# CrispyChillies/Image-Retrieval---Thesis-2026

Measured on AMD Instinct MI355X. Metric: queries/sec (embed+top-10) over 1M x 1024 gallery, higher is better.
Workload: dtype f32 embed (two fp16 MFMA terms); bf16 MFMA candidates + f64 re-rank

## Files before the change

image-retrieval---thesis-2026_amd/_lib.py:

```python
import ctypes
import os

_HERE = os.path.dirname(os.path.abspath(__file__))
LIB_PATH = os.environ.get("MIRX_LIB_PATH", os.path.join(_HERE, "libmirx.so"))

METRIC_IP = 0
ESTATE = -4
METRIC_NEG_L2 = 1
TIER_AUTO = 0
TIER_EXACT_ONLY = 3
OPT_TIERS = 1
OPT_SAMPLE_RANK = 2
OPT_FORCE_TAU = 3
OPT_PROFILE = 4
OPT_RANK_SORT = 5
OPT_COMPACT_CHUNK_ROWS = 6
OPT_MASK_GATHER_BYTES = 7
OPT_RANGE_MAX_HITS = 8
RANK_SORT_AUTO = 0
RANK_SORT_BITONIC = 1
RANK_SORT_RADIX = 2
MAX_SEARCH_K = 1024
GROUP_MAX_LIMIT, GROUP_MAX_SIZE, GROUP_MAX_HITS, GROUP_FILL_MAX = 1024, 64, 16384, 4096
FUSE_MAX_REQUESTS, FUSE_MAX_ENTRIES, FUSE_MAX_LIMIT = 8, 4096, 1024
FUSE_RRF, FUSE_WEIGHTED = 0, 1
FUSE_NORMS = {"RAW": 0, "COSINE": 1, "IP": 2, "L2": 3}
TUNE_CONV1X1_SMALL_MAX_WG = 1
TUNE_CONV3X3_SMALL_MAX_WG = 2
TUNE_CONV1X1_RING = 3
SIMCAM_MAPS_BOTH = 0
SIMCAM_MAPS_RETRIEVED = 1
SIMATT_GROUP = 0
SIMATT_PAIRS = 1
ANOMALY_BAD_SCORE = 1
ANOMALY_BAD_NORM = 2
ANOMALY_BAD_ONE_CLASS = 4
ANOMALY_BAD_EMPTY_CLASS = 8
RESAMPLE_MAX_SIDE = 8192
RESAMPLE_MAX_TAPS = 65
RESAMPLE_MAX_OUT = 1024
RESAMPLE_MAX_BATCH = 65536
RESAMPLE_MAX_LDS = 65536
RESAMPLE_TILE_W, RESAMPLE_TILE_H = 32, 16
RESAMPLE_DESC_WORDS = 8
RESAMPLE_OUT_U8, RESAMPLE_OUT_F32 = 0, 1
RESAMPLE_BILINEAR, RESAMPLE_BICUBIC = 0, 1
IVF_MAX_NLIST, IVF_MAX_DIM = 65536, 2048
IVF_FLAT, IVF_SQ8 = 0, 1
IVF_PQ = 2
PQ_MAX_M = 64
IVF_OPT_SCORE_BYTES = 1
ROLLOUT_FUSE = {"mean": 0, "max": 1, "min": 2}
STAGES = ("prep", "sample", "gemm", "finalize", "exact")
FORCE_TAU_OFF = 0x7FC00000


class MirxError(RuntimeError):
    """A libmirx call failed (message from mirx_last_error())."""


class SearchStats(ctypes.Structure):
    _fields_ = [(n, ctypes.c_int64) for n in
                ("nq", "tier1_answered", "exact_answered", "candidates", "reranked",
                 "overflowed", "incomplete", "left_out")]

    def as_dict(self):
        return {n: int(getattr(self, n)) for n, _ in self._fields_}


class RangeStats(ctypes.Structure):
    _fields_ = [(n, ctypes.c_int64) for n in ("nq", "filter_answered", "exact_answered", "candidates", "hits")]

    def as_dict(self):
        return {n: int(getattr(self, n)) for n, _ in self._fields_}


class IvfStats(ctypes.Structure):
    _fields_ = [(n, ctypes.c_int64) for n in ("nq", "rows_scored", "pairs", "work_items", "batches")]

    def as_dict(self):
        return {n: int(getattr(self, n)) for n, _ in self._fields_}


_vp, _i64, _int = ctypes.c_void_p, ctypes.c_int64, ctypes.c_int
SYMBOLS = {
    "mirx_last_error": (ctypes.c_char_p, []),
    "mirx_version": (_int, []),
    "mirx_set_tuning": (_int, [_int, _i64]),
    "mirx_index_create": (_int, [_int, _int, _int, ctypes.POINTER(_vp)]),
    "mirx_index_destroy": (None, [_vp]),
    "mirx_index_add": (_int, [_vp, _vp, _i64, _vp]),
    "mirx_index_reserve": (_int, [_vp, _i64]),
    "mirx_index_size": (_i64, [_vp]),
    "mirx_index_dim": (_int, [_vp]),
    "mirx_index_set_option": (_int, [_vp, _int, _i64]),
    "mirx_index_get_rows": (_int, [_vp, _i64, _i64, _vp, _vp]),
    "mirx_index_remove_ids": (_int, [_vp, _vp, _i64, ctypes.POINTER(_i64), _vp]),
    "mirx_compact_tile": (_int, []),
    "mirx_index_search": (_int, [_vp, _vp, _i64, _int, _vp, _vp, _vp, _vp]),
    "mirx_index_search_f64": (_int, [_vp, _vp, _i64, _int, _vp, _vp, _vp, _vp]),
    "mirx_index_search_begin": (_int, [_vp, _vp, _i64, _int, _vp, _vp, _vp, _vp, _vp]),
    "mirx_index_search_end": (_int, [_vp]),
    "mirx_index_search_masked": (_int, [_vp, _vp, _i64, _int, _vp, _vp, _i64, _vp, _vp, _vp, _vp]),
    "mirx_index_search_deep": (_int, [_vp, _vp, _i64, _int, _vp, _vp, _vp, _vp, _vp, _vp]),
    "mirx_index_search_leave_out": (_int, [_vp, _vp, _i64, _int, _vp, _vp, _vp, _vp, _i64, _vp, _vp, _vp, _vp]),
    "mirx_tier1_max_k": (_int, []),
    "mirx_deep_min_rows": (_i64, [_int, _i64]),
    "mirx_index_rank_top_masked": (_int, [_vp, _vp, _i64, _i64, _vp, _vp, _i64, _vp, _vp, _vp, _vp]),
    "mirx_index_range_search": (_int, [_vp, _vp, _i64, ctypes.c_double, ctypes.c_double, _vp, _vp, _i64, _vp,
                                       ctypes.POINTER(_i64), _vp]),
    "mirx_index_range_fetch": (_int, [_vp, _vp, _vp, _vp, _vp]),
    "mirx_index_range_last_stats": (_int, [_vp, ctypes.POINTER(RangeStats)]),
# ... 201 lines not shown
```

image-retrieval---thesis-2026_amd/csrc/k_stem_h2.hip:

```cpp
#include "mirx_device.h"
#include "mirx_kernels.h"

namespace mirx {

namespace {

constexpr int PTH = 8, PTW = 7;
constexpr int CTH = 2 * PTH + 1;
constexpr int CTW = 2 * PTW + 1;
constexpr int NPX = CTH * CTW;
constexpr int ITH = 2 * (CTH - 1) + 7;
constexpr int ITW = 2 * (CTW - 1) + 7;
constexpr int PH = 24;
constexpr int PLANE = 3 * ITH * PH;
constexpr int OCB = 32;
constexpr int NOB = 2;
constexpr int NSTEP = 11;
constexpr int CONV_PITCH = 260;
constexpr int S_IN = 2 * PLANE;
constexpr int S_CONV = OCB * CONV_PITCH;
constexpr int W_BYTES = NOB * NSTEP * 2 * OCB * 16 * 2;
constexpr int STEP_BYTES = NOB * 2 * 1024;
constexpr int RING_OFF = S_IN * 4;
#if defined(MIRX_STEM_NCH) && !defined(MIRX_DIAG)
#error "MIRX_STEM_NCH without -DMIRX_DIAG: the shipped library carries one ring depth"
#endif
#ifndef MIRX_STEM_NCH
#define MIRX_STEM_NCH 2
#endif
constexpr int par_off(int nch) { return RING_OFF + 2 * nch * STEP_BYTES; }
constexpr int lds_bytes(int nch) { return par_off(nch) + 4 * NOB * OCB * 4; }
constexpr int wg_per_cu(int nch) { return 160 * 1024 / lds_bytes(nch) > 4 ? 4 : 160 * 1024 / lds_bytes(nch); }
static_assert(lds_bytes(2) <= 40960, "NCH = 2: four workgroups per CU");

__device__ inline void split2h_pair_cvt(float a, float b, unsigned &h, unsigned &l) {
    const f32x2 v = {a, b};
    const f16x2 vh = __builtin_convertvector(v, f16x2);
    const f32x2 r1 = v - __builtin_convertvector(vh, f32x2);
    const f16x2 vl = __builtin_convertvector(r1, f16x2);
    h = __builtin_bit_cast(unsigned, vh);
    l = __builtin_bit_cast(unsigned, vl);
}

template <typename TIN, int NCH>
__global__ __launch_bounds__(256, wg_per_cu(NCH)) void k_stem_h2(const TIN *__restrict__ x, const uint16_t *__restrict__ w3,
                                                                 const float *__restrict__ oscale, const float *__restrict__ scale,
                                                                 const float *__restrict__ shift, int h, int wd,
                                                                 float *__restrict__ y, int64_t y_bs,
                                                                 const float *__restrict__ in_range, unsigned *__restrict__ out_range,
                                                                 const float *__restrict__ mean, const float *__restrict__ stdv) {
    extern __shared__ __attribute__((aligned(16))) float sm[];
    constexpr bool U8 = sizeof(TIN) == 1;
    constexpr int NCHUNK = (NSTEP + NCH - 1) / NCH;
    constexpr int RING_BUF = NCH * STEP_BYTES;
    constexpr int PAR_OFF = par_off(NCH);
    static_assert(S_CONV * 4 <= PAR_OFF, "the conv tile of a channel block lies over the patch and the ring");
    static_assert(!U8 || 768 * 4 <= RING_BUF, "the 8-bit table lies in ring buffer 1");
    char *s_ring = reinterpret_cast<char *>(sm) + RING_OFF;
    float *s_lut = reinterpret_cast<float *>(s_ring + RING_BUF);
    if (U8) {
        for (int i = threadIdx.x; i < 768; i += 256) s_lut[i] = ((float)(i & 255) / 255.0f - mean[i >> 8]) / stdv[i >> 8];
        __syncthreads();
    }
    float *s_in = sm;
    float *s_conv = sm;
    const int ph = h / 4, pw = wd / 4, ch = h / 2, cw = wd / 2;
    const int tiles_x = (pw + PTW - 1) / PTW;
    int tile = blockIdx.x;
    int64_t img = blockIdx.y;
#ifndef MIRX_STEM_PLAIN_ORDER
    {
        const unsigned ntile = gridDim.x, lin = blockIdx.x + ntile * blockIdx.y, full = gridDim.y & ~7u;
        if (lin < ntile * full) {
            const unsigned j = lin >> 3;
            tile = (int)(j % ntile);
            img = (int64_t)(j / ntile) * 8 + (lin & 7);
        }
    }
#endif
    const int tile_y = tile / tiles_x, tile_x = tile % tiles_x;
    const int oc0 = 0;
    const int py0 = tile_y * PTH, px0 = tile_x * PTW;
    const int cy0 = 2 * py0 - 1, cx0 = 2 * px0 - 1;
    const int iy0 = 2 * cy0 - 3, ix0 = 2 * cx0 - 3;
    const TIN *xi = x + img * 3 * (int64_t)h * wd;
    float x_scale, x_inv;
    range_scales(in_range[img], x_scale, x_inv);
    float *s_par = sm + PAR_OFF / 4;
    if (threadIdx.x < NOB * OCB) {
        s_par[4 * threadIdx.x] = oscale[threadIdx.x] * x_inv;
        s_par[4 * threadIdx.x + 1] = scale[threadIdx.x];
        s_par[4 * threadIdx.x + 2] = shift[threadIdx.x];
    }

#ifndef MIRX_STEM_EXP
#define MIRX_STEM_EXP 0
#endif
    const int dwv = __builtin_amdgcn_readfirstlane(threadIdx.x >> 6);
    const __amdgpu_buffer_rsrc_t wrsrc = __builtin_amdgcn_make_buffer_rsrc((void *)w3, 0, W_BYTES, 0x00020000);
    const int dvoff = ((threadIdx.x & 63) >> 1) * 32 + (((threadIdx.x & 1) ^ ((threadIdx.x >> 4) & 1)) << 4);
    auto issue_chunk = [&](int c) {
        if (MIRX_STEM_EXP & 8) return;
#pragma unroll
        for (int j = 0; j < NCH; ++j) {
            const int s = c * NCH + j;
            if (s < NSTEP)
                __builtin_amdgcn_raw_ptr_buffer_load_lds(wrsrc, LDS_PTR(s_ring + (c & 1) * RING_BUF + j * STEP_BYTES + dwv * 1024), 16,
                                                         dvoff, ((dwv >> 1) * NSTEP * 2 + s * 2 + (dwv & 1)) * 1024, 0, 0);
        }
    };
    issue_chunk(0);
    if (!U8 && NCHUNK > 1) issue_chunk(1);

    constexpr int ROWW = 36, RPP = 7;
    constexpr int N_IN = (3 * ITH + RPP - 1) / RPP;
    const int s_row = threadIdx.x / ROWW, s_q = threadIdx.x % ROWW;
    const int xx = ix0 + s_q;
    const bool col_ok = s_row < RPP && s_q < ITW && xx >= 0 && xx < wd;
    const bool lane_live = s_row < RPP;
    float vin[N_IN];
#pragma unroll
    for (int t = 0; t < N_IN; ++t) {
        const int row = RPP * t + s_row;
        const int c = (row >= ITH) + (row >= 2 * ITH), r = row - c * ITH;
        const int yy = iy0 + r;
        vin[t] = 0.0f;
        if (col_ok && row < 3 * ITH && yy >= 0 && yy < h) {
            if constexpr (U8) vin[t] = s_lut[c * 256 + xi[((int64_t)c * h + yy) * wd + xx]];
            else vin[t] = xi[((int64_t)c * h + yy) * wd + xx];
        }
    }
    unsigned *s_w = reinterpret_cast<unsigned *>(s_in);
    const int s_dst = (s_q & 1) * PLANE + s_row * PH + (s_q >> 1);
#pragma unroll
    for (int t = 0; t < N_IN; ++t) {
        const float v = vin[t] * x_scale;
        const _Float16 vh = (_Float16)v;
        const _Float16 vl = (_Float16)(v - (float)vh);
        const unsigned word = (unsigned)__builtin_bit_cast(unsigned short, vh) | ((unsigned)__builtin_bit_cast(unsigned short, vl) << 16);
        if (lane_live && RPP * t + s_row < 3 * ITH) s_w[s_dst + RPP * t * PH] = word;
    }
    asm volatile("s_waitcnt vmcnt(0)" ::: "memory");
    __syncthreads();
    if (U8 && NCHUNK > 1) issue_chunk(1);

    const int wave = threadIdx.x >> 6, lane = threadIdx.x & 63;
    const int half = lane >> 5, n = lane & 31;
    int xbase[2];
#pragma unroll
    for (int t = 0; t < 2; ++t) {
        int p = (2 * wave + t) * 32 + n;
        if (p >= NPX) p = NPX - 1;
        const int r = p / CTW, q = p % CTW;
        xbase[t] = 2 * r * PH + q;
    }
    const char *wp = s_ring + n * 32 + ((half ^ ((n >> 3) & 1)) << 4);
    f32x16 acc[2][NOB];
#pragma unroll
    for (int t = 0; t < 2; ++t)
#pragma unroll
        for (int b = 0; b < NOB; ++b)
#pragma unroll
            for (int r = 0; r < 16; ++r) acc[t][b][r] = 0.0f;
#pragma unroll
    for (int c = 0; c < ((MIRX_STEM_EXP & 1) ? 0 : NCHUNK); ++c) {
        if (c > 0 && c + 1 < NCHUNK) issue_chunk(c + 1);
        __builtin_amdgcn_sched_barrier(0);
        const char *wc = wp + (c & 1) * RING_BUF;
#pragma unroll
        for (int j = 0; j < NCH; ++j) {
            const int s = c * NCH + j;
            if (s >= NSTEP) break;
            f16x8 ah[NOB], al[NOB];
#pragma unroll
            for (int b = 0; b < NOB; ++b) {
                ah[b] = *reinterpret_cast<const f16x8 *>(wc + j * STEP_BYTES + (b * 2 + 0) * 1024);
                al[b] = *reinterpret_cast<const f16x8 *>(wc + j * STEP_BYTES + (b * 2 + 1) * 1024);
            }
            const int rho0 = 2 * s, rho1 = 2 * s + 1 < 21 ? 2 * s + 1 : 20;
            const int ro0 = ((rho0 / 7) * ITH + rho0 % 7) * PH, ro1 = ((rho1 / 7) * ITH + rho1 % 7) * PH;
            const int ro = half ? ro1 : ro0;
#pragma unroll
            for (int t = 0; t < 2; ++t) {
                const unsigned *pe = s_w + xbase[t] + ro;
                const unsigned *po = pe + PLANE;
                u32x4 bh, bl;
                bh[0] = __builtin_amdgcn_perm(pe[1], pe[0], 0x05040100u); bl[0] = __builtin_amdgcn_perm(pe[1], pe[0], 0x07060302u);
                bh[1] = __builtin_amdgcn_perm(pe[3], pe[2], 0x05040100u); bl[1] = __builtin_amdgcn_perm(pe[3], pe[2], 0x07060302u);
                bh[2] = __builtin_amdgcn_perm(po[1], po[0], 0x05040100u); bl[2] = __builtin_amdgcn_perm(po[1], po[0], 0x07060302u);
                bh[3] = __builtin_amdgcn_perm(po[3], po[2], 0x05040100u); bl[3] = __builtin_amdgcn_perm(po[3], po[2], 0x07060302u);
                const f16x8 xh = __builtin_bit_cast(f16x8, bh), xl = __builtin_bit_cast(f16x8, bl);
#pragma unroll
                for (int b = 0; b < NOB; ++b) {
                    f32x16 a3 = acc[t][b];
                    a3 = __builtin_amdgcn_mfma_f32_32x32x16_f16(al[b], xh, a3, 0, 0, 0);
                    a3 = __builtin_amdgcn_mfma_f32_32x32x16_f16(ah[b], xl, a3, 0, 0, 0);
                    a3 = __builtin_amdgcn_mfma_f32_32x32x16_f16(ah[b], xh, a3, 0, 0, 0);
                    acc[t][b] = a3;
                }
                __builtin_amdgcn_sched_barrier(0);
            }
        }
        if (c + 1 < NCHUNK) {
            asm volatile("s_waitcnt vmcnt(0)" ::: "memory");
            __syncthreads();
        }
    }

    asm volatile("s_waitcnt vmcnt(0)" ::: "memory");
    int pp[2];
    bool live[2], inside[2];
#pragma unroll
    for (int t = 0; t < 2; ++t) {
        pp[t] = (2 * wave + t) * 32 + n;
        live[t] = pp[t] < NPX;
        const int r0 = pp[t] / CTW, q = pp[t] % CTW;
        const int cy = cy0 + r0, cx = cx0 + q;
        inside[t] = cy >= 0 && cy < ch && cx >= 0 && cx < cw;
    }
    float *yi = y + img * y_bs + oc0 * (int64_t)ph * pw;
    float vmax = 0.f;
#pragma unroll
    for (int b = 0; b < NOB; ++b) {
        __syncthreads();
        if (!(MIRX_STEM_EXP & 2)) {
#pragma unroll
            for (int r = 0; r < 16; ++r) {
                const int ocl = 8 * (r >> 2) + (r & 3) + 4 * half;
                const f32x4 pr = *reinterpret_cast<const f32x4 *>(s_par + 4 * (b * OCB + ocl));
#pragma unroll
                for (int t = 0; t < 2; ++t) {
                    const float v = fmaxf(fmaf(acc[t][b][r] * pr[0], pr[1], pr[2]), 0.0f);
                    if (live[t]) s_conv[ocl * CONV_PITCH + pp[t]] = inside[t] ? v : 0.0f;
                }
            }
        }
        __syncthreads();
        for (int i = threadIdx.x; i < ((MIRX_STEM_EXP & 4) ? 0 : OCB * PTH * 8); i += 256) {
            const int ocl = i / (PTH * 8), r = (i / 8) % PTH, q = i % 8;
            const int py = py0 + r, px = px0 + q;
            if (q < PTW && py < ph && px < pw) {
                const float *cbase = s_conv + ocl * CONV_PITCH + (2 * r) * CTW + 2 * q;
                float m = 0.0f;
#pragma unroll
                for (int dy = 0; dy < 3; ++dy)
#pragma unroll
                    for (int dx = 0; dx < 3; ++dx) m = fmaxf(m, cbase[dy * CTW + dx]);
                if (x_inv != x_inv) m = x_inv;
                yi[((int64_t)(b * OCB + ocl) * ph + py) * pw + px] = m;
                vmax = range_max(vmax, m);
            }
        }
    }
    if (out_range) range_publish(out_range, (int)img, vmax, threadIdx.x & 63);
}

template <typename TIN>
static hipError_t launch_stem_h2_t(const TIN *x, const uint16_t *w2, const float *oscale, const float *scale, const float *shift,
                                   int64_t n, int h, int wd, float *y, int64_t y_bs, const float *in_range, float *out_range,
                                   const float *mean, const float *stdv, hipStream_t st) {
    if (n <= 0) return hipSuccess;
    if (n > 65535 || !in_range || !oscale) return hipErrorInvalidValue;
    const int ph = h / 4, pw = wd / 4;
    const int tiles = ((ph + PTH - 1) / PTH) * ((pw + PTW - 1) / PTW);
    constexpr int NCH = MIRX_STEM_NCH;
    const size_t lds = lds_bytes(NCH);
    static std::atomic<unsigned long long> attr_devs{0};
    hipError_t e = set_dynamic_lds(k_stem_h2<TIN, NCH>, lds, &attr_devs);
    if (e != hipSuccess) return e;
    hipLaunchKernelGGL((k_stem_h2<TIN, NCH>), dim3((unsigned)tiles, (unsigned)n, 1), dim3(256), lds, st, x, w2, oscale, scale, shift,
                       h, wd, y, y_bs, in_range, reinterpret_cast<unsigned *>(out_range), mean, stdv);
    return hipGetLastError();
}

}

hipError_t launch_stem_h2(const float *x, const uint16_t *w2, const float *oscale, const float *scale, const float *shift,
                          int64_t n, int h, int wd, float *y, int64_t y_bs, const float *in_range, float *out_range,
                          hipStream_t st) {
    return launch_stem_h2_t<float>(x, w2, oscale, scale, shift, n, h, wd, y, y_bs, in_range, out_range, nullptr, nullptr, st);
}

hipError_t launch_stem_h2_u8(const uint8_t *x, const float *mean, const float *stdv, const uint16_t *w2, const float *oscale,
                             const float *scale, const float *shift, int64_t n, int h, int wd, float *y, int64_t y_bs,
                             const float *in_range, float *out_range, hipStream_t st) {
    if (!mean || !stdv) return hipErrorInvalidValue;
    return launch_stem_h2_t<uint8_t>(x, w2, oscale, scale, shift, n, h, wd, y, y_bs, in_range, out_range, mean, stdv, st);
}

namespace {
__global__ __launch_bounds__(256) void k_range_absmax(const float *__restrict__ x, int64_t per, unsigned *__restrict__ row) {
    const float *xi = x + (int64_t)blockIdx.y * per;
    float m = 0.f;
    if ((reinterpret_cast<uintptr_t>(xi) & 15) == 0) {
        const int64_t nv = per >> 2;
        for (int64_t i = (int64_t)blockIdx.x * 256 + threadIdx.x; i < nv; i += (int64_t)gridDim.x * 256) {
            const f32x4 v = reinterpret_cast<const f32x4 *>(xi)[i];
            m = range_max(range_max(range_max(range_max(m, v[0]), v[1]), v[2]), v[3]);
        }
        if (blockIdx.x == 0 && threadIdx.x < (per & 3)) m = range_max(m, xi[(nv << 2) + threadIdx.x]);
    } else {
        for (int64_t i = (int64_t)blockIdx.x * 256 + threadIdx.x; i < per; i += (int64_t)gridDim.x * 256) m = range_max(m, xi[i]);
    }
    range_publish(row, (int)blockIdx.y, m, threadIdx.x & 63);
}
}

namespace {
__global__ __launch_bounds__(256) void k_range_absmax_u8(const uint8_t *__restrict__ x, int64_t hw, const float *__restrict__ mean,
                                                         const float *__restrict__ stdv, unsigned *__restrict__ row) {
    __shared__ float s_lut[768];
    for (int i = threadIdx.x; i < 768; i += 256) s_lut[i] = ((float)(i & 255) / 255.0f - mean[i >> 8]) / stdv[i >> 8];
    __syncthreads();
    const uint8_t *xi = x + (int64_t)blockIdx.y * 3 * hw;
    float m = 0.f;
    for (int c = 0; c < 3; ++c)
        for (int64_t i = (int64_t)blockIdx.x * 256 + threadIdx.x; i < hw; i += (int64_t)gridDim.x * 256)
            m = range_max(m, s_lut[c * 256 + xi[c * hw + i]]);
    range_publish(row, (int)blockIdx.y, m, threadIdx.x & 63);
}
}

hipError_t launch_range_absmax_u8(const uint8_t *x, int64_t hw, int64_t n, const float *mean, const float *stdv, float *row,
                                  hipStream_t st) {
    if (n <= 0 || hw <= 0) return hipSuccess;
    if (n > 65535 || !mean || !stdv) return hipErrorInvalidValue;
    const int64_t want = (hw + 255) / 256;
    const unsigned chunks = (unsigned)(want > 16 ? 16 : want);
    hipLaunchKernelGGL(k_range_absmax_u8, dim3(chunks, (unsigned)n), dim3(256), 0, st, x, hw, mean, stdv, reinterpret_cast<unsigned *>(row));
    return hipGetLastError();
}

hipError_t launch_range_absmax(const float *x, int64_t per, int64_t n, float *row, hipStream_t st) {
    if (n <= 0 || per <= 0) return hipSuccess;
    if (n > 65535) return hipErrorInvalidValue;
    const int64_t want = (per / 4 + 16 * 256 - 1) / (16 * 256);
    const unsigned chunks = (unsigned)(want < 1 ? 1 : (want > 16 ? 16 : want));
    hipLaunchKernelGGL(k_range_absmax, dim3(chunks, (unsigned)n), dim3(256), 0, st, x, per, reinterpret_cast<unsigned *>(row));
    return hipGetLastError();
}

}
```

image-retrieval---thesis-2026_amd/csrc/mirx_api.hip:

```cpp
#include <algorithm>
#include <cmath>
#include <cstring>
#include <vector>

#include "mirx_kernels.h"

namespace mirx {

static thread_local std::string g_err;
void set_error(const std::string &msg) { g_err = msg; }
int fail(int code, const std::string &msg) {
    g_err = msg;
    return code;
}

constexpr int64_t QUERY_BATCH = 8192;
constexpr int64_t TIER1_MIN_ROWS = 32768;
constexpr int TIER1_MAX_K = 64;

}

using namespace mirx;

extern "C" {

const char *mirx_last_error(void) { return g_err.c_str(); }
int mirx_version(void) { return MIRX_VERSION; }

int mirx_set_tuning(int key, int64_t value) {
    switch (key) {
        case MIRX_TUNE_CONV1X1_SMALL_MAX_WG:
            MIRX_CHECK(value >= 0 && value <= (1 << 20), "set_tuning: conv1x1 small-launch limit out of range");
            set_conv1x1_small_max_wg((int)value);
            return MIRX_OK;
        case MIRX_TUNE_CONV3X3_SMALL_MAX_WG:
            MIRX_CHECK(value >= 0 && value <= (1 << 20), "set_tuning: conv3x3 small-launch limit out of range");
            set_conv3x3_small_max_wg((int)value);
            return MIRX_OK;
        case MIRX_TUNE_CONV1X1_RING:
            MIRX_CHECK(value == 0 || value == 1, "set_tuning: conv1x1 ring switch must be 0 or 1");
            set_conv1x1_ring((int)value);
            return MIRX_OK;
        default:
            return fail(MIRX_EINVAL, "set_tuning: unknown key");
    }
}

int mirx_compact_tile(void) { return COMPACT_TILE; }
uint64_t mirx_rank_key(double score) { return rank_key(score); }
int mirx_rank_sort_tile(void) { return RANK_TILE; }

int mirx_topk_merge(const double *in_scores, const int64_t *in_ids, int nshard, int64_t nq, int k,
                    int metric, double *out_rank_scores, float *out_scores, int64_t *out_ids, void *stream) {
    MIRX_CHECK(in_scores && in_ids && out_ids && nshard >= 1 && nq >= 0 && k >= 1, "topk_merge: bad argument");
    MIRX_CHECK((int64_t)nshard * k <= 8192, "topk_merge: nshard * k must be <= 8192");
    MIRX_HIP(launch_topk_merge(in_scores, in_ids, nshard, nq, k, metric, out_rank_scores, out_scores,
                               out_ids, reinterpret_cast<hipStream_t>(stream)));
    return MIRX_OK;
}

int mirx_conv1x1_bn_relu_split3(const float *x, int64_t x_batch_stride, int cin, const float *scale1_or_null,
                                const float *shift1_or_null, const void *w3, const float *bias_or_null, int64_t n,
                                int hw, int cout, int relu_out, float *y, int64_t y_batch_stride, void *stream) {
    MIRX_CHECK(n >= 0 && hw >= 1 && cin >= 16 && cin % 16 == 0 && cout >= 128 && cout % 128 == 0,
               "conv1x1_split3: cin must be a multiple of 16 and cout of 128");
    MIRX_CHECK((scale1_or_null == nullptr) == (shift1_or_null == nullptr), "conv1x1_split3: scale and shift go together");
    MIRX_CHECK(n == 0 || (x && w3 && y), "conv1x1_split3: null buffer");
    MIRX_CHECK(x_batch_stride >= (int64_t)cin * hw, "conv1x1_split3: batch stride smaller than the channel prefix");
    MIRX_CHECK(y_batch_stride >= (int64_t)cout * hw, "conv1x1_split3: output batch stride smaller than cout * hw");
    MIRX_HIP(launch_conv1x1_s3(x, x_batch_stride, cin, scale1_or_null, shift1_or_null,
                               reinterpret_cast<const uint16_t *>(w3), bias_or_null, n, hw, cout, relu_out, y,
                               y_batch_stride, reinterpret_cast<hipStream_t>(stream)));
    return MIRX_OK;
}

int mirx_conv1x1_bn_relu_split2h(const float *x, int64_t x_batch_stride, int cin, const float *scale1_or_null,
                                 const float *shift1_or_null, const void *w2, const float *oscale,
                                 const float *bias_or_null, int64_t n, int hw, int cout, int relu_out, float *y,
                                 int64_t y_batch_stride, const float *in_range_or_null, float in_ks, float in_kb,
                                 float *out_range_or_null, int64_t x_plane_stride, int64_t y_plane_stride, void *stream) {
    MIRX_CHECK(n >= 0 && hw >= 1 && cin >= 16 && cin % 16 == 0 && cout >= 128 && cout % 128 == 0,
               "conv1x1_split2h: cin must be a multiple of 16 and cout of 128");
    if (!x_plane_stride) x_plane_stride = hw;
    if (!y_plane_stride) y_plane_stride = hw;
    MIRX_CHECK(x_plane_stride >= hw && y_plane_stride >= hw, "conv1x1_split2h: a plane stride is 0 (= hw) or at least hw");
    MIRX_CHECK((scale1_or_null == nullptr) == (shift1_or_null == nullptr), "conv1x1_split2h: scale and shift go together");
    MIRX_CHECK(n == 0 || (x && w2 && y && oscale), "conv1x1_split2h: null buffer");
    MIRX_CHECK(x_batch_stride >= (int64_t)cin * x_plane_stride, "conv1x1_split2h: batch stride smaller than the channel prefix");
    MIRX_CHECK(y_batch_stride >= (int64_t)cout * y_plane_stride, "conv1x1_split2h: output batch stride smaller than cout planes");
    MIRX_CHECK(in_ks >= 0.f && in_kb >= 0.f && (in_range_or_null || in_kb > 0.f),
               "conv1x1_split2h: in_ks / in_kb are non-negative; without range slots in_kb is the bound itself");
    MIRX_HIP(launch_conv1x1_h2(x, x_batch_stride, cin, scale1_or_null, shift1_or_null,
                               reinterpret_cast<const uint16_t *>(w2), oscale, bias_or_null, n, hw, cout, relu_out, y,
                               y_batch_stride, in_range_or_null, in_ks, in_kb, out_range_or_null, 0.f, 0.f, nullptr,
                               x_plane_stride, y_plane_stride, reinterpret_cast<hipStream_t>(stream)));
    return MIRX_OK;
}


int mirx_conv1x1_bn_relu_split2h_terms(const float *x, int64_t x_batch_stride, int cin, const float *scale1,
                                       const float *shift1, const void *w2, const float *oscale, const float *bias,
                                       int64_t n, int hw, void *y_terms, const float *in_range, float in_ks, float in_kb,
                                       float y_ks, float y_kb, float *y_inv_out, int64_t x_plane_stride, void *stream) {
    MIRX_CHECK(n >= 0 && hw >= 1 && cin >= 16 && cin % 16 == 0, "conv1x1_split2h_terms: cin must be a multiple of 16");
    MIRX_CHECK(n == 0 || (x && w2 && y_terms && oscale && scale1 && shift1 && bias && in_range && y_inv_out),
               "conv1x1_split2h_terms: null buffer");
    if (!x_plane_stride) x_plane_stride = hw;
    MIRX_CHECK(x_plane_stride >= hw, "conv1x1_split2h_terms: the plane stride is 0 (= hw) or at least hw");
    MIRX_CHECK(x_batch_stride >= (int64_t)cin * x_plane_stride, "conv1x1_split2h_terms: batch stride smaller than the channel prefix");
    MIRX_CHECK(in_ks >= 0.f && in_kb >= 0.f && y_ks >= 0.f && y_kb >= 0.f, "conv1x1_split2h_terms: bounds are non-negative");
    MIRX_HIP(launch_conv1x1_h2(x, x_batch_stride, cin, scale1, shift1, reinterpret_cast<const uint16_t *>(w2), oscale, bias, n,
                               hw, 128, 1, reinterpret_cast<float *>(y_terms), 0, in_range, in_ks, in_kb, nullptr, y_ks, y_kb,
                               y_inv_out, x_plane_stride, 0, reinterpret_cast<hipStream_t>(stream)));
    return MIRX_OK;
}

int mirx_conv3x3_direct_terms_nchw(const void *y_terms, const void *w2, const float *oscale, int64_t n, int side, float *out,
                                   int64_t out_batch_stride, const float *y_inv, float *out_range_or_null,
                                   int64_t out_plane_stride, void *stream) {
    MIRX_CHECK(n >= 0 && n <= 65535, "conv3x3_terms: batch must be in [0, 65535]");
    MIRX_CHECK(side == 56 || side == 28 || side == 14 || side == 7, "conv3x3_terms: side must be 56, 28, 14 or 7");
    MIRX_CHECK(n == 0 || (y_terms && w2 && oscale && out && y_inv), "conv3x3_terms: null buffer");
    if (!out_plane_stride) out_plane_stride = (int64_t)side * side;
    MIRX_CHECK(out_plane_stride >= (int64_t)side * side, "conv3x3_terms: the plane stride is 0 (= side^2) or at least side^2");
// ... 836 lines not shown
```

image-retrieval---thesis-2026_amd/csrc/mirx_kernels.h:

```cpp
#pragma once
#include "mirx_common.h"

namespace mirx {

extern const int64_t QUERY_BATCH;
extern const int64_t TIER1_MIN_ROWS;
extern const int TIER1_MAX_K;

hipError_t launch_ingest(const float *src, int64_t n, int dim, int dimp, float *g32,
                         uint16_t *g16, float *gbias, unsigned *gnorm_max_bits, int metric,
                         hipStream_t st);
hipError_t launch_prep_queries(const float *q, int64_t nq, int64_t nq_pad, int dim, int dimp,
                               float *q32p, uint16_t *q16, float *qnorm, hipStream_t st);
hipError_t launch_l2_normalize(float *x, int64_t n, int dim, hipStream_t st);
hipError_t launch_bn_relu_gap_l2norm(const float *x, const float *scale, const float *shift,
                                     int64_t n, int c, int hw, int normalize, float *y,
                                     hipStream_t st);
hipError_t launch_bn_relu_nchw(const float *x, int64_t x_batch_stride, const float *scale,
                               const float *shift, int64_t n, int c, int hw, float *y, hipStream_t st);
hipError_t launch_bn_relu_avgpool2(const float *x, int64_t x_batch_stride, const float *scale,
                                   const float *shift, int64_t n, int c, int h, int w, float *y,
                                   int64_t x_plane_stride, hipStream_t st, int64_t y_batch_stride = 0);
hipError_t launch_stem(const float *x, const float *w, const float *scale, const float *shift,
                       int64_t n, int h, int wd, float *y, hipStream_t st);
hipError_t launch_stem_s3(const float *x, const uint16_t *w3, const float *scale, const float *shift, int64_t n, int h,
                          int wd, float *y, int64_t y_bs, float *out_range, hipStream_t st);

hipError_t launch_stem_h2(const float *x, const uint16_t *w2, const float *oscale, const float *scale, const float *shift,
                          int64_t n, int h, int wd, float *y, int64_t y_bs, const float *in_range, float *out_range,
                          hipStream_t st);
hipError_t launch_range_absmax(const float *x, int64_t per_image, int64_t n, float *row, hipStream_t st);
hipError_t launch_stem_h2_u8(const uint8_t *x, const float *mean, const float *stdv, const uint16_t *w2, const float *oscale,
                             const float *scale, const float *shift, int64_t n, int h, int wd, float *y, int64_t y_bs,
                             const float *in_range, float *out_range, hipStream_t st);
hipError_t launch_range_absmax_u8(const uint8_t *x, int64_t hw, int64_t n, const float *mean, const float *stdv, float *row,
                                  hipStream_t st);

hipError_t launch_conv1x1(const float *x, int64_t xbs, int cin, const float *scale, const float *shift,
                          const float *wt, const float *bias, int64_t n, int hw, int cout, int relu_out, float *y,
                          hipStream_t st);

hipError_t launch_dwconv7_nhwc(const float *x, const float *wt, const float *bias, int64_t n, int c, int h, int wd, float *y,
                               hipStream_t st);
hipError_t launch_dwconv7(const float *x, const float *w, const float *bias, int64_t n, int c, int h, int wd,
                          float *y, hipStream_t st);
hipError_t launch_grn_norm(const float *x, int64_t n, int hw, int c, float *gx, hipStream_t st);
hipError_t launch_grn_scale(const float *gx, const float *weight, int64_t n, int c, float eps, float *scale, float *smax,
                            hipStream_t st);

hipError_t launch_scores_f64(const float *q32p, const int32_t *qlist, int nq, const float *g32,
                             int64_t n, int dimp, int metric, double *out, int64_t ld,
                             hipStream_t st);
hipError_t launch_row_topk(const double *scores, int64_t ld, int64_t n, const int64_t *ids,
                           const int32_t *qlist, int nq, const int64_t *exclude, int k,
                           int metric, double *out_f64, int64_t *out_ids, float *out_val,
                           hipStream_t st);
hipError_t launch_rank_rows(const double *scores, int64_t ld, int64_t n, const int64_t *ids,
                            const int64_t *exclude, int nq, Hit *work, int64_t np2, int metric,
                            int64_t *out_ids, float *out_val, hipStream_t st);
hipError_t launch_topk_merge(const double *in_scores, const int64_t *in_ids, int nshard,
                             int64_t nq, int k, int metric, double *out_f64, float *out_val,
                             int64_t *out_ids, hipStream_t st);

int64_t rank_sort_tiles(int64_t n);
hipError_t launch_rank_sort_build(const double *scores, int64_t ld, int64_t n, const int64_t *ids, const int32_t *perm,
                                  const int64_t *exclude, int drop_excluded, int nq, uint64_t *keys, int32_t *pay, hipStream_t st);
hipError_t launch_rank_sort_build_ids(const int64_t *ids, int64_t n, uint64_t *keys, int32_t *pay, hipStream_t st);
hipError_t launch_rank_sort(uint64_t *keys_a, int32_t *pay_a, uint64_t *keys_b, int32_t *pay_b, unsigned *hist, int64_t n,
                            int nseg, hipStream_t st, int key_bits = 64);
hipError_t launch_rank_sort_write(const int32_t *pay, int64_t n, int64_t kout, const double *scores, int64_t ld,
                                  const int64_t *ids, const int64_t *exclude, int drop_excluded, int metric, int nq,
                                  int64_t *out_ids, float *out_val, double *out_f64, hipStream_t st);

int64_t compact_tiles(int64_t n);
size_t compact_scratch_bytes(int64_t chunk_rows, int dimp);
hipError_t launch_compact_scan(const int64_t *ids, int64_t n, const uint64_t *req, int64_t nreq, int32_t *pos, int32_t *part,
                               hipStream_t st);
hipError_t launch_compact_scan_flags(int32_t *pos, int64_t n, int32_t *part, hipStream_t st);
hipError_t launch_compact_gather(const float *g32, const int64_t *ids, const int32_t *pos, int64_t n, int dimp, float *s32,
                                 int64_t *sid, hipStream_t st);
hipError_t launch_compact_chunk(float *g32, uint16_t *g16, int64_t *ids, float *gbias, void *scratch, int64_t chunk_rows,
                                const int32_t *pos, int64_t c0, int64_t c1, int dimp, hipStream_t st);

hipError_t launch_mask_pass(const uint8_t *allow, int64_t n, int64_t cap, const float *gbias, const int64_t *ids, float *bias,
                            int64_t *mids, int32_t *pos, int32_t *part, hipStream_t st);
hipError_t launch_mask_scores(double *scores, int64_t ld, int64_t n, const int32_t *pos, int nq, hipStream_t st);
hipError_t launch_leave_out_scores(double *scores, int64_t ld, int64_t n, const int32_t *row_codes, const int32_t *query_codes,
                                   const int32_t *qlist, int nq, hipStream_t st);
hipError_t launch_mask_gather_codes(const int32_t *row_codes, const int32_t *pos, int64_t n, int32_t *out, hipStream_t st);
hipError_t launch_mask_rank_keys(uint64_t *keys, const int32_t *pay, int64_t n, const uint8_t *allow, int nq, hipStream_t st);
hipError_t launch_mask_rank_tail(const int32_t *pay, int64_t n, int64_t kout, const uint8_t *allow, int nq, int64_t *out_ids,
                                 float *out_val, double *out_f64, hipStream_t st);

int64_t an_chunk_rows(int64_t n, int d);
int64_t class_centroids_workspace_bytes(int64_t n, int d, int k);
hipError_t launch_class_centroids(const float *rows, int64_t n, int d, const int64_t *labels, const int64_t *classes_host, int k,
                                  void *workspace, double *centroids, int64_t *counts, int *bad, hipStream_t st);
hipError_t launch_centroid_min_dist(const float *rows, int64_t n, int d, const double *centroids, int k, double *dist,
                                    int32_t *nearest, double *max_out, hipStream_t st);
int64_t binary_rank_metrics_workspace_bytes(int64_t nseg, int64_t n);
hipError_t launch_binary_rank_metrics(const double *scores, const uint8_t *positive, int64_t nseg, int64_t n, const double *norm,
                                      double level, void *workspace, double *thresholds, int64_t *tps, int64_t *fps, int64_t *out_t,
                                      double *out_auroc, double *out_aupr, double *out_fpr, int *bad, hipStream_t st);

int64_t insdel_steps_workspace_bytes(int64_t k, int64_t hw);
hipError_t launch_insdel_steps(const float *sal, int64_t k, int64_t hw, int64_t step, void *workspace, int32_t *t, hipStream_t st);
int64_t blur2d_blocks(int64_t planes, int h, int w);
hipError_t launch_blur2d_same(const float *x, int64_t planes, int h, int w, const float *kern, int klen, float *y, hipStream_t st);
hipError_t launch_insdel_compose(const int32_t *t, int64_t n_rows, int64_t hw, const float *bank, int64_t n_bank, const int32_t *start,
                                 const int32_t *finish, const int32_t *row, int64_t n_steps, int64_t g0, int64_t n, float *out,
                                 hipStream_t st);
hipError_t launch_insdel_curves(const float *q, const float *r, int64_t n_curves, int64_t n_steps, int d, double *scores, double *auc,
                                int64_t *zero_counter, hipStream_t st);
// ... 383 lines not shown
```

include/mirx.h:

```cpp
#ifndef MIRX_H
#define MIRX_H

#include <stdint.h>

#ifdef __cplusplus
extern "C" {
#endif

#define MIRX_VERSION 305

#define MIRX_OK 0
#define MIRX_EINVAL (-1)
#define MIRX_ENOMEM (-2)
#define MIRX_EHIP (-3)
#define MIRX_ESTATE (-4)

#define MIRX_METRIC_IP 0
#define MIRX_METRIC_NEG_L2 1

#define MIRX_TIER_AUTO 0
#define MIRX_TIER_EXACT_ONLY 3

#define MIRX_OPT_TIERS 1
#define MIRX_OPT_SAMPLE_RANK 2
#define MIRX_OPT_FORCE_TAU 3
#define MIRX_OPT_PROFILE 4
#define MIRX_OPT_RANK_SORT 5
#define MIRX_OPT_COMPACT_CHUNK_ROWS 6
#define MIRX_OPT_MASK_GATHER_BYTES 7
#define MIRX_OPT_RANGE_MAX_HITS 8

#define MIRX_RANK_SORT_AUTO 0
#define MIRX_RANK_SORT_BITONIC 1
#define MIRX_RANK_SORT_RADIX 2

#define MIRX_STAGE_PREP 0
#define MIRX_STAGE_SAMPLE 1
#define MIRX_STAGE_GEMM 2
#define MIRX_STAGE_FINALIZE 3
#define MIRX_STAGE_EXACT 4
#define MIRX_NUM_STAGES 5

typedef struct mirx_index mirx_index;

typedef struct mirx_search_stats {
    int64_t nq;
    int64_t tier1_answered;
    int64_t exact_answered;
    int64_t candidates;
    int64_t reranked;
    int64_t overflowed;
    int64_t incomplete;
    int64_t left_out;
} mirx_search_stats;

const char *mirx_last_error(void);
int mirx_version(void);

#define MIRX_TUNE_CONV1X1_SMALL_MAX_WG 1
#define MIRX_TUNE_CONV3X3_SMALL_MAX_WG 2
#define MIRX_TUNE_CONV1X1_RING 3
int mirx_set_tuning(int key, int64_t value);

int mirx_index_create(int dim, int metric, int device, mirx_index **out);
void mirx_index_destroy(mirx_index *ix);

int mirx_index_add(mirx_index *ix, const float *rows, int64_t n, const int64_t *ids_or_null);
int mirx_index_reserve(mirx_index *ix, int64_t capacity_rows);
int64_t mirx_index_size(const mirx_index *ix);
int mirx_index_dim(const mirx_index *ix);
int mirx_index_set_option(mirx_index *ix, int option, int64_t value);

int mirx_index_get_rows(const mirx_index *ix, int64_t first, int64_t n, float *out_rows,
                        int64_t *out_ids_or_null);

int mirx_index_remove_ids(mirx_index *ix, const int64_t *ids, int64_t n, int64_t *out_removed_or_null, void *stream);
int mirx_compact_tile(void);

int mirx_index_search(mirx_index *ix, const float *q, int64_t nq, int k,
                      const int64_t *exclude_ids_or_null, float *out_scores, int64_t *out_ids,
                      void *stream);

int mirx_index_search_f64(mirx_index *ix, const float *q, int64_t nq, int k,
                          const int64_t *exclude_ids_or_null, double *out_rank_scores,
                          int64_t *out_ids, void *stream);

int mirx_index_search_begin(mirx_index *ix, const float *q, int64_t nq, int k, const int64_t *exclude_ids_or_null,
                            float *out_scores_or_null, double *out_rank_scores_or_null, int64_t *out_ids, void *stream);
int mirx_index_search_end(mirx_index *ix);

int mirx_index_search_masked(mirx_index *ix, const float *q, int64_t nq, int k, const int64_t *exclude_ids_or_null,
                             const uint8_t *allow, int64_t n_allow, float *out_scores_or_null,
                             double *out_rank_scores_or_null, int64_t *out_ids, void *stream);

int mirx_index_search_deep(mirx_index *ix, const float *queries, int64_t nq, int k, const int64_t *exclude_ids_or_null,
                           const uint8_t *allow_or_null, float *out_values_or_null, double *out_f64_or_null, int64_t *out_ids,
                           void *stream);
int mirx_tier1_max_k(void);
int64_t mirx_deep_min_rows(int k_eff, int64_t nq);

int mirx_index_search_leave_out(mirx_index *ix, const float *queries, int64_t nq, int k, const int64_t *exclude_ids_or_null,
                                const uint8_t *allow_or_null, const int32_t *row_codes, const int32_t *query_codes,
                                int64_t max_left_out, float *out_values_or_null, double *out_f64_or_null, int64_t *out_ids,
                                void *stream);

typedef struct mirx_range_stats {
    int64_t nq;
    int64_t filter_answered;
    int64_t exact_answered;
    int64_t candidates;
    int64_t hits;
} mirx_range_stats;

int mirx_index_range_search(mirx_index *ix, const float *q, int64_t nq, double lo, double hi, const int64_t *exclude_ids_or_null,
                            const uint8_t *allow_or_null, int64_t n_allow, int64_t *out_lims, int64_t *out_total, void *stream);
int mirx_index_range_fetch(mirx_index *ix, float *out_values_or_null, double *out_f64_or_null, int64_t *out_ids, void *stream);
int mirx_index_range_last_stats(mirx_index *ix, mirx_range_stats *out);

int mirx_index_last_stats(mirx_index *ix, void *stream, mirx_search_stats *out);

int mirx_index_last_timings(mirx_index *ix, float *out_ms);

int mirx_index_rank_all(mirx_index *ix, const float *q, int64_t nq,
                        const int64_t *exclude_ids_or_null, int64_t *out_ids,
                        float *out_scores_or_null, void *stream);

int mirx_index_rank_top(mirx_index *ix, const float *q, int64_t nq, int64_t k, const int64_t *exclude_ids_or_null,
                        float *out_scores_or_null, double *out_rank_scores_or_null, int64_t *out_ids, void *stream);

int mirx_index_rank_top_masked(mirx_index *ix, const float *q, int64_t nq, int64_t k, const int64_t *exclude_ids_or_null,
                               const uint8_t *allow, int64_t n_allow, float *out_scores_or_null,
                               double *out_rank_scores_or_null, int64_t *out_ids, void *stream);

uint64_t mirx_rank_key(double score);
int mirx_rank_sort_tile(void);

int mirx_topk_merge(const double *in_scores, const int64_t *in_ids, int nshard, int64_t nq,
                    int k, int metric, double *out_rank_scores, float *out_scores,
                    int64_t *out_ids, void *stream);

int mirx_conv1x1_bn_relu_split3(const float *x, int64_t x_batch_stride, int cin, const float *scale1_or_null,
                                const float *shift1_or_null, const void *w3, const float *bias_or_null,
                                int64_t n, int hw, int cout, int relu_out, float *y, int64_t y_batch_stride,
                                void *stream);
// ... 450 lines not shown
```

Baseline: 45060.

## Rework stem patch LDS layout for bank-conflict-free reads, default 7x8 tile

Templates the stem kernel geometry on pool tile shape and switches the default from 8x7 to 7x8 pooled pixels. It also replaces the padded patch layout with a row-pair layout whose bank-conflict freedom is checked at compile time. The max-pool epilogue now writes four outputs per thread as one float4 store. The aim is fewer LDS bank conflicts and fewer, wider global stores in the stem conv. The cost is more template instantiations and index math, plus a new tuning switch to fall back to the old tile shape.

```diff
diff --git a/image-retrieval---thesis-2026_amd/_lib.py b/image-retrieval---thesis-2026_amd/_lib.py
--- a/image-retrieval---thesis-2026_amd/_lib.py
+++ b/image-retrieval---thesis-2026_amd/_lib.py
@@ -28,6 +28,7 @@
 TUNE_CONV1X1_SMALL_MAX_WG = 1
 TUNE_CONV3X3_SMALL_MAX_WG = 2
 TUNE_CONV1X1_RING = 3
+TUNE_STEM_TILE = 4
 SIMCAM_MAPS_BOTH = 0
 SIMCAM_MAPS_RETRIEVED = 1
 SIMATT_GROUP = 0
diff --git a/image-retrieval---thesis-2026_amd/csrc/k_stem_h2.hip b/image-retrieval---thesis-2026_amd/csrc/k_stem_h2.hip
--- a/image-retrieval---thesis-2026_amd/csrc/k_stem_h2.hip
+++ b/image-retrieval---thesis-2026_amd/csrc/k_stem_h2.hip
@@ -5,33 +5,126 @@
 
 namespace {
 
-constexpr int PTH = 8, PTW = 7;
-constexpr int CTH = 2 * PTH + 1;
-constexpr int CTW = 2 * PTW + 1;
-constexpr int NPX = CTH * CTW;
-constexpr int ITH = 2 * (CTH - 1) + 7;
-constexpr int ITW = 2 * (CTW - 1) + 7;
-constexpr int PH = 24;
-constexpr int PLANE = 3 * ITH * PH;
 constexpr int OCB = 32;
 constexpr int NOB = 2;
 constexpr int NSTEP = 11;
-constexpr int CONV_PITCH = 260;
-constexpr int S_IN = 2 * PLANE;
-constexpr int S_CONV = OCB * CONV_PITCH;
 constexpr int W_BYTES = NOB * NSTEP * 2 * OCB * 16 * 2;
 constexpr int STEP_BYTES = NOB * 2 * 1024;
-constexpr int RING_OFF = S_IN * 4;
 #if defined(MIRX_STEM_NCH) && !defined(MIRX_DIAG)
 #error "MIRX_STEM_NCH without -DMIRX_DIAG: the shipped library carries one ring depth"
 #endif
 #ifndef MIRX_STEM_NCH
 #define MIRX_STEM_NCH 2
 #endif
-constexpr int par_off(int nch) { return RING_OFF + 2 * nch * STEP_BYTES; }
-constexpr int lds_bytes(int nch) { return par_off(nch) + 4 * NOB * OCB * 4; }
-constexpr int wg_per_cu(int nch) { return 160 * 1024 / lds_bytes(nch) > 4 ? 4 : 160 * 1024 / lds_bytes(nch); }
-static_assert(lds_bytes(2) <= 40960, "NCH = 2: four workgroups per CU");
+
+template <int PTH_, int PTW_>
+struct StemGeo {
+    static constexpr int PTH = PTH_, PTW = PTW_;
+    static constexpr int CTH = 2 * PTH + 1;
+    static constexpr int CTW = 2 * PTW + 1;
+    static constexpr int NPX = CTH * CTW;
+    static constexpr int ITH = 2 * (CTH - 1) + 7;
+    static constexpr int ITW = 2 * (CTW - 1) + 7;
+    static constexpr int ROWW = ITW + 1;
+    static constexpr int RPP = 256 / ROWW;
+    static constexpr int N_IN = (3 * ITH + RPP - 1) / RPP;
+    static constexpr int HW = ROWW / 2;
+    static constexpr int P2 = (2 * HW - CTW + 31) / 32 * 32 + CTW;
+    static constexpr int ODD = HW;
+    static constexpr int CPL = (ITH + 1) / 2 * P2;
+    static constexpr int PLANE = (3 * CPL + 15) / 32 * 32 + 16;
+    static constexpr int S_IN = 2 * PLANE;
+    static constexpr int CONV_PITCH = NPX;
+    static constexpr int S_CONV = OCB * CONV_PITCH;
+    static constexpr int RING_OFF = S_IN * 4;
+    static constexpr int NQ = (PTW + 3) / 4;
+    static constexpr int par_off(int nch) { return RING_OFF + 2 * nch * STEP_BYTES; }
+    static constexpr int lds_bytes(int nch) { return par_off(nch) + 4 * NOB * OCB * 4; }
+    static constexpr int wg_per_cu(int nch) { return 160 * 1024 / lds_bytes(nch) > 4 ? 4 : 160 * 1024 / lds_bytes(nch); }
+    static constexpr int patch_word(int c, int rho, int q) { return (q & 1) * PLANE + c * CPL + (rho >> 1) * P2 + (rho & 1) * ODD + (q >> 1); }
+    static_assert(NPX == 255 && CONV_PITCH % 2 == 1, "eight 32-pixel column blocks, one idle lane");
+    static_assert(ODD >= HW && P2 - ODD >= HW && P2 % 32 == CTW % 32, "the rows of a pair do not overlap; conv rows CTW banks apart");
+    static_assert(RING_OFF % 16 == 0, "the ring is read with ds_read_b128");
+    static_assert(lds_bytes(2) <= 40960, "NCH = 2: four workgroups per CU");
+};
+
+constexpr int group_ways(const int *addr, const bool *on) {
+    int cnt[32] = {};
+    int worst = 0;
+    for (int i = 0; i < 32; ++i) {
+        if (!on[i]) continue;
+        bool dup = false;
+        for (int j = 0; j < i; ++j) dup = dup || (on[j] && addr[j] == addr[i]);
+        if (dup) continue;
+        const int b = ((addr[i] % 32) + 32) % 32;
+        if (++cnt[b] > worst) worst = cnt[b];
+    }
+    return worst;
+}
+template <class G>
+constexpr int stage_store_ways() {
+    int worst = 0;
+    for (int t = 0; t < G::N_IN; ++t)
+        for (int g = 0; g < 8; ++g) {
+            int addr[32] = {};
+            bool on[32] = {};
+            for (int l = 0; l < 32; ++l) {
+                const int tid = 32 * g + l, slot = tid / G::ROWW, q = tid % G::ROWW, row = G::RPP * t + slot;
+                on[l] = slot < G::RPP && row < 3 * G::ITH;
+                if (on[l]) addr[l] = G::patch_word(row / G::ITH, row % G::ITH, q);
+            }
+            const int w = group_ways(addr, on);
+            if (w > worst) worst = w;
+        }
+    return worst;
+}
+template <class G>
+constexpr int b_read_ways() {
+    int worst = 0;
+    for (int k = 0; k < 8; ++k) {
+        int addr[32] = {};
+        bool on[32] = {};
+        for (int n = 0; n < 32; ++n) {
+            const int p = 32 * k + n < G::NPX ? 32 * k + n : G::NPX - 1;
+            on[n] = true;
+            addr[n] = (p / G::CTW) * G::P2 + p % G::CTW;
+        }
+        const int w = group_ways(addr, on);
+        if (w > worst) worst = w;
+    }
+    return worst;
+}
+template <class G>
+constexpr int conv_store_ways() {
+    int worst = 0;
+    for (int k = 0; k < 8; ++k) {
+        int addr[32] = {};
+        bool on[32] = {};
+        for (int n = 0; n < 32; ++n) {
+            on[n] = 32 * k + n < G::NPX;
+            addr[n] = 32 * k + n;
+        }
+        const int w = group_ways(addr, on);
+        if (w > worst) worst = w;
+    }
+    return worst;
+}
+template <class G>
+constexpr int pool_read_ways() {
+    int addr[32] = {};
+    bool on[32] = {};
+    for (int l = 0; l < 32; ++l) {
+        on[l] = true;
+        addr[l] = l * G::CONV_PITCH;
+    }
+    return group_ways(addr, on);
+}
+template <class G>
+constexpr bool banking_holds() {
+    return b_read_ways<G>() == 1 && pool_read_ways<G>() == 1 && conv_store_ways<G>() == 1 && stage_store_ways<G>() <= 2;
+}
+static_assert(banking_holds<StemGeo<7, 8>>(), "<7, 8>: reads and conv-tile stores conflict-free, staging stores at most 2-way (free)");
+static_assert(banking_holds<StemGeo<8, 7>>(), "<8, 7>: the same");
 
 __device__ inline void split2h_pair_cvt(float a, float b, unsigned &h, unsigned &l) {
     const f32x2 v = {a, b};
@@ -42,18 +135,19 @@
     l = __builtin_bit_cast(unsigned, vl);
 }
 
-template <typename TIN, int NCH>
-__global__ __launch_bounds__(256, wg_per_cu(NCH)) void k_stem_h2(const TIN *__restrict__ x, const uint16_t *__restrict__ w3,
-                                                                 const float *__restrict__ oscale, const float *__restrict__ scale,
-                                                                 const float *__restrict__ shift, int h, int wd,
-                                                                 float *__restrict__ y, int64_t y_bs,
-                                                                 const float *__restrict__ in_range, unsigned *__restrict__ out_range,
-                                                                 const float *__restrict__ mean, const float *__restrict__ stdv) {
+template <typename TIN, int NCH, int PTH, int PTW>
+__global__ __launch_bounds__(256, (StemGeo<PTH, PTW>::wg_per_cu(NCH))) void k_stem_h2(
+    const TIN *__restrict__ x, const uint16_t *__restrict__ w3, const float *__restrict__ oscale, const float *__restrict__ scale,
+    const float *__restrict__ shift, int h, int wd, float *__restrict__ y, int64_t y_bs, const float *__restrict__ in_range,
+    unsigned *__restrict__ out_range, const float *__restrict__ mean, const float *__restrict__ stdv) {
+    using G = StemGeo<PTH, PTW>;
+    constexpr int CTW = G::CTW, NPX = G::NPX, ITH = G::ITH, ITW = G::ITW, P2 = G::P2, ODD = G::ODD, CPL = G::CPL, PLANE = G::PLANE;
+    constexpr int CONV_PITCH = G::CONV_PITCH, S_CONV = G::S_CONV, RING_OFF = G::RING_OFF;
     extern __shared__ __attribute__((aligned(16))) float sm[];
     constexpr bool U8 = sizeof(TIN) == 1;
     constexpr int NCHUNK = (NSTEP + NCH - 1) / NCH;
     constexpr int RING_BUF = NCH * STEP_BYTES;
-    constexpr int PAR_OFF = par_off(NCH);
+    constexpr int PAR_OFF = G::par_off(NCH);
     static_assert(S_CONV * 4 <= PAR_OFF, "the conv tile of a channel block lies over the patch and the ring");
     static_assert(!U8 || 768 * 4 <= RING_BUF, "the 8-bit table lies in ring buffer 1");
     char *s_ring = reinterpret_cast<char *>(sm) + RING_OFF;
@@ -112,8 +206,8 @@
     issue_chunk(0);
     if (!U8 && NCHUNK > 1) issue_chunk(1);
 
-    constexpr int ROWW = 36, RPP = 7;
-    constexpr int N_IN = (3 * ITH + RPP - 1) / RPP;
+    constexpr int ROWW = G::ROWW, RPP = G::RPP;
+    constexpr int N_IN = G::N_IN;
     const int s_row = threadIdx.x / ROWW, s_q = threadIdx.x % ROWW;
     const int xx = ix0 + s_q;
     const bool col_ok = s_row < RPP && s_q < ITW && xx >= 0 && xx < wd;
@@ -131,14 +225,16 @@
         }
     }
     unsigned *s_w = reinterpret_cast<unsigned *>(s_in);
-    const int s_dst = (s_q & 1) * PLANE + s_row * PH + (s_q >> 1);
+    const int s_dst = (s_q & 1) * PLANE + (s_q >> 1);
 #pragma unroll
     for (int t = 0; t < N_IN; ++t) {
         const float v = vin[t] * x_scale;
         const _Float16 vh = (_Float16)v;
         const _Float16 vl = (_Float16)(v - (float)vh);
         const unsigned word = (unsigned)__builtin_bit_cast(unsigned short, vh) | ((unsigned)__builtin_bit_cast(unsigned short, vl) << 16);
-        if (lane_live && RPP * t + s_row < 3 * ITH) s_w[s_dst + RPP * t * PH] = word;
+        const int row = RPP * t + s_row;
+        const int c = (row >= ITH) + (row >= 2 * ITH), r = row - c * ITH;
+        if (lane_live && row < 3 * ITH) s_w[s_dst + c * CPL + (r >> 1) * P2 + (r & 1) * ODD] = word;
     }
     asm volatile("s_waitcnt vmcnt(0)" ::: "memory");
     __syncthreads();
@@ -152,7 +248,7 @@
         int p = (2 * wave + t) * 32 + n;
         if (p >= NPX) p = NPX - 1;
         const int r = p / CTW, q = p % CTW;
-        xbase[t] = 2 * r * PH + q;
+        xbase[t] = r * P2 + q;
     }
     const char *wp = s_ring + n * 32 + ((half ^ ((n >> 3) & 1)) << 4);
     f32x16 acc[2][NOB];
@@ -178,7 +274,7 @@
                 al[b] = *reinterpret_cast<const f16x8 *>(wc + j * STEP_BYTES + (b * 2 + 1) * 1024);
             }
             const int rho0 = 2 * s, rho1 = 2 * s + 1 < 21 ? 2 * s + 1 : 20;
-            const int ro0 = ((rho0 / 7) * ITH + rho0 % 7) * PH, ro1 = ((rho1 / 7) * ITH + rho1 % 7) * PH;
+            const int ro0 = G::patch_word(rho0 / 7, rho0 % 7, 0), ro1 = G::patch_word(rho1 / 7, rho1 % 7, 0);
             const int ro = half ? ro1 : ro0;
 #pragma unroll
             for (int t = 0; t < 2; ++t) {
@@ -236,24 +332,59 @@
             }
         }
         __syncthreads();
-        for (int i = threadIdx.x; i < ((MIRX_STEM_EXP & 4) ? 0 : OCB * PTH * 8); i += 256) {
-            const int ocl = i / (PTH * 8), r = (i / 8) % PTH, q = i % 8;
-            const int py = py0 + r, px = px0 + q;
-            if (q < PTW && py < ph && px < pw) {
-                const float *cbase = s_conv + ocl * CONV_PITCH + (2 * r) * CTW + 2 * q;
-                float m = 0.0f;
-#pragma unroll
-                for (int dy = 0; dy < 3; ++dy)
-#pragma unroll
-                    for (int dx = 0; dx < 3; ++dx) m = fmaxf(m, cbase[dy * CTW + dx]);
-                if (x_inv != x_inv) m = x_inv;
-                yi[((int64_t)(b * OCB + ocl) * ph + py) * pw + px] = m;
-                vmax = range_max(vmax, m);
+        constexpr int NQ = G::NQ;
+        for (int i = threadIdx.x; i < ((MIRX_STEM_EXP & 4) ? 0 : OCB * PTH * NQ); i += 256) {
+            const int ocl = i & (OCB - 1), r = (i >> 5) / NQ, qd = (i >> 5) % NQ;
+            const int py = py0 + r, px = px0 + 4 * qd;
+            if (py < ph && px < pw) {
+                const float *cbase = s_conv + ocl * CONV_PITCH + (2 * r) * CTW + 8 * qd;
+                float cm[9];
+#pragma unroll
+                for (int dx = 0; dx < 9; ++dx) {
+                    const int d = 8 * (NQ - 1) + dx < CTW ? dx : min(dx, CTW - 1 - 8 * qd);
+                    cm[dx] = fmaxf(fmaxf(cbase[d], cbase[CTW + d]), cbase[2 * CTW + d]);
+                }
+                f32x4 m;
+#pragma unroll
+                for (int k = 0; k < 4; ++k) {
+                    m[k] = fmaxf(fmaxf(fmaxf(0.0f, cm[2 * k]), cm[2 * k + 1]), cm[2 * k + 2]);
+                    if (x_inv != x_inv) m[k] = x_inv;
+                }
+                const int nv = min(min(PTW - 4 * qd, pw - px), 4);
+                float *dst = yi + ((int64_t)(b * OCB + ocl) * ph + py) * pw + px;
+                if (nv == 4 && (reinterpret_cast<uintptr_t>(dst) & 15) == 0) {
+                    *reinterpret_cast<f32x4 *>(dst) = m;
+                } else {
+#pragma unroll
+                    for (int k = 0; k < 4; ++k)
+                        if (k < nv) dst[k] = m[k];
+                }
+#pragma unroll
+                for (int k = 0; k < 4; ++k)
+                    if (k < nv) vmax = range_max(vmax, m[k]);
             }
         }
     }
     if (out_range) range_publish(out_range, (int)img, vmax, threadIdx.x & 63);
 }
+
+template <typename TIN, int PTH, int PTW>
+static hipError_t launch_stem_h2_arm(const TIN *x, const uint16_t *w2, const float *oscale, const float *scale, const float *shift,
+                                     int64_t n, int h, int wd, float *y, int64_t y_bs, const float *in_range, float *out_range,
+                                     const float *mean, const float *stdv, hipStream_t st) {
+    const int ph = h / 4, pw = wd / 4;
+    const int tiles = ((ph + PTH - 1) / PTH) * ((pw + PTW - 1) / PTW);
+    constexpr int NCH = MIRX_STEM_NCH;
+    const size_t lds = StemGeo<PTH, PTW>::lds_bytes(NCH);
+    static std::atomic<unsigned long long> attr_devs{0};
+    hipError_t e = set_dynamic_lds(k_stem_h2<TIN, NCH, PTH, PTW>, lds, &attr_devs);
+    if (e != hipSuccess) return e;
+    hipLaunchKernelGGL((k_stem_h2<TIN, NCH, PTH, PTW>), dim3((unsigned)tiles, (unsigned)n, 1), dim3(256), lds, st, x, w2, oscale,
+                       scale, shift, h, wd, y, y_bs, in_range, reinterpret_cast<unsigned *>(out_range), mean, stdv);
+    return hipGetLastError();
+}
+
+std::atomic<int> g_stem_tile{1};
 
 template <typename TIN>
 static hipError_t launch_stem_h2_t(const TIN *x, const uint16_t *w2, const float *oscale, const float *scale, const float *shift,
@@ -261,19 +392,14 @@
                                    const float *mean, const float *stdv, hipStream_t st) {
     if (n <= 0) return hipSuccess;
     if (n > 65535 || !in_range || !oscale) return hipErrorInvalidValue;
-    const int ph = h / 4, pw = wd / 4;
-    const int tiles = ((ph + PTH - 1) / PTH) * ((pw + PTW - 1) / PTW);
-    constexpr int NCH = MIRX_STEM_NCH;
-    const size_t lds = lds_bytes(NCH);
-    static std::atomic<unsigned long long> attr_devs{0};
-    hipError_t e = set_dynamic_lds(k_stem_h2<TIN, NCH>, lds, &attr_devs);
-    if (e != hipSuccess) return e;
-    hipLaunchKernelGGL((k_stem_h2<TIN, NCH>), dim3((unsigned)tiles, (unsigned)n, 1), dim3(256), lds, st, x, w2, oscale, scale, shift,
-                       h, wd, y, y_bs, in_range, reinterpret_cast<unsigned *>(out_range), mean, stdv);
-    return hipGetLastError();
-}
-
-}
+    if (g_stem_tile.load(std::memory_order_relaxed))
+        return launch_stem_h2_arm<TIN, 7, 8>(x, w2, oscale, scale, shift, n, h, wd, y, y_bs, in_range, out_range, mean, stdv, st);
+    return launch_stem_h2_arm<TIN, 8, 7>(x, w2, oscale, scale, shift, n, h, wd, y, y_bs, in_range, out_range, mean, stdv, st);
+}
+
+}
+
+void set_stem_tile(int v) { g_stem_tile.store(v ? 1 : 0); }
 
 hipError_t launch_stem_h2(const float *x, const uint16_t *w2, const float *oscale, const float *scale, const float *shift,
                           int64_t n, int h, int wd, float *y, int64_t y_bs, const float *in_range, float *out_range,
diff --git a/image-retrieval---thesis-2026_amd/csrc/mirx_api.hip b/image-retrieval---thesis-2026_amd/csrc/mirx_api.hip
--- a/image-retrieval---thesis-2026_amd/csrc/mirx_api.hip
+++ b/image-retrieval---thesis-2026_amd/csrc/mirx_api.hip
@@ -40,6 +40,10 @@
         case MIRX_TUNE_CONV1X1_RING:
             MIRX_CHECK(value == 0 || value == 1, "set_tuning: conv1x1 ring switch must be 0 or 1");
             set_conv1x1_ring((int)value);
+            return MIRX_OK;
+        case MIRX_TUNE_STEM_TILE:
+            MIRX_CHECK(value == 0 || value == 1, "set_tuning: stem tile switch must be 0 or 1");
+            set_stem_tile((int)value);
             return MIRX_OK;
         default:
             return fail(MIRX_EINVAL, "set_tuning: unknown key");
diff --git a/image-retrieval---thesis-2026_amd/csrc/mirx_kernels.h b/image-retrieval---thesis-2026_amd/csrc/mirx_kernels.h
--- a/image-retrieval---thesis-2026_amd/csrc/mirx_kernels.h
+++ b/image-retrieval---thesis-2026_amd/csrc/mirx_kernels.h
@@ -29,6 +29,7 @@
 hipError_t launch_stem_h2(const float *x, const uint16_t *w2, const float *oscale, const float *scale, const float *shift,
                           int64_t n, int h, int wd, float *y, int64_t y_bs, const float *in_range, float *out_range,
                           hipStream_t st);
+void set_stem_tile(int v);
 hipError_t launch_range_absmax(const float *x, int64_t per_image, int64_t n, float *row, hipStream_t st);
 hipError_t launch_stem_h2_u8(const uint8_t *x, const float *mean, const float *stdv, const uint16_t *w2, const float *oscale,
                              const float *scale, const float *shift, int64_t n, int h, int wd, float *y, int64_t y_bs,
diff --git a/include/mirx.h b/include/mirx.h
--- a/include/mirx.h
+++ b/include/mirx.h
@@ -60,6 +60,7 @@
 #define MIRX_TUNE_CONV1X1_SMALL_MAX_WG 1
 #define MIRX_TUNE_CONV3X3_SMALL_MAX_WG 2
 #define MIRX_TUNE_CONV1X1_RING 3
+#define MIRX_TUNE_STEM_TILE 4
 int mirx_set_tuning(int key, int64_t value);
 
 int mirx_index_create(int dim, int metric, int device, mirx_index **out);
```

Result: no change. 45380 (median of 5 runs) (+0.7%).
